# mbrzus/Cross-Modality-Minipig-Gan

Hardware: AMD Instinct MI355X
Metric: T1->T2 256x256 slices/sec (G+D step) (higher is better)
Workload: dtype f32

## Files before the change

cross-modality-minipig-gan_amd/csrc/conv_igemm.hip:

```cpp
#include "mpgan_common.h"
#include "conv_geom.h"
#include "lds_dma.h"
#include "conv_pipe.h"
#include <stdlib.h>
#include <algorithm>
#include <type_traits>

namespace mpgan {


struct KCursor {
  int ci, jz, jy, jx;
  int delta;
  int dz, dy, dx;
  int woff;
  bool valid;
};

template <int BN, int TM, int TN, int WN, bool SCALAR>
__global__ __launch_bounds__(256) void gather_conv_kernel(const GatherConv p) {
  extern __shared__ __attribute__((aligned(16))) float lds[];
  constexpr int STAGE = (BM + BN) * PITCH;
  constexpr int BROWS = BN / 32;

// ... 657 lines not shown
  const int T = p.Kz * p.Ky * p.Kx;
  for (int i = threadIdx.x; i < T * p.Cin; i += 256) wl[i] = p.wp[i];
  __syncthreads();
  const unsigned Mtot = (unsigned)p.N * ph.Mz * ph.My * ph.Mx;
  const unsigned gi = blockIdx.x * 256u + threadIdx.x;
  const unsigned m = gi / LANES;
  const int l = (int)(gi % LANES);
  const bool live = m < Mtot;
  PixDecode d = decode_pixel(p, ph, live ? m : 0u);
  float acc = 0.f;
  if (live && d.opix >= 0) {
    for (int jz = 0; jz < ph.nz; ++jz) {
      const int iz = d.bz + ph.dz0 + p.dstep[0] * jz, kz = ph.kz0 + p.kstep[0] * jz;
      if ((unsigned)iz >= (unsigned)p.Di) continue;
      for (int jy = 0; jy < ph.ny; ++jy) {
        const int iy = d.by + ph.dy0 + p.dstep[1] * jy, ky = ph.ky0 + p.kstep[1] * jy;
        if ((unsigned)iy >= (unsigned)p.Hi) continue;
        const long rowbase = (((long)d.n * p.Di + iz) * p.Hi + iy) * p.Wi;
        for (int jx = 0; jx < ph.nx; ++jx) {
          const int ix = d.bx + ph.dx0 + p.dstep[2] * jx, kx = ph.kx0 + p.kstep[2] * jx;
          if ((unsigned)ix >= (unsigned)p.Wi) continue;
          float4 v;
          if constexpr (IN_BF16) {
            typedef __bf16 bf16x4 __attribute__((ext_vector_type(4)));
            const bf16x4 t = *reinterpret_cast<const bf16x4*>(reinterpret_cast<const __bf16*>(p.in) + (rowbase + ix) * p.ldi + 4 * l);
            v = make_float4((float)t[0], (float)t[1], (float)t[2], (float)t[3]);
          } else {
            v = *reinterpret_cast<const float4*>(p.in + (rowbase + ix) * p.ldi + 4 * l);
          }
          const float4 w = *reinterpret_cast<const float4*>(wl + ((kz * p.Ky + ky) * p.Kx + kx) * p.Cin + 4 * l);
          acc = fmaf(v.x, w.x, acc);
          acc = fmaf(v.y, w.y, acc);
          acc = fmaf(v.z, w.z, acc);
          acc = fmaf(v.w, w.w, acc);
        }
      }
    }
  }
#pragma unroll
  for (int off = LANES / 2; off > 0; off >>= 1) acc += __shfl_xor(acc, off, 64);
  if (live && d.opix >= 0 && l == 0) {
    float v = acc + (p.bias ? p.bias[0] : 0.f);
    if (p.epi.scale) v = epi_act1(v, p.epi.scale[0], p.epi.shift[0], p.epi.slope[0]);
    if (p.resid) v += p.resid[(long)d.opix * p.ldr];
    if (p.tanh_out) v = tanhf(v);
    p.out[(long)d.opix * p.ldo] = v;
  }
}

template <int LANES>
__global__ __launch_bounds__(256) void convt_quad_cout1_kernel(const GatherConv p) {
  extern __shared__ __attribute__((aligned(16))) float wl[];
  const int Cin = p.Cin;
  for (int i = threadIdx.x; i < 9 * Cin; i += 256) wl[i] = p.wp[i];
  __syncthreads();
  const Phase& ph = p.ph[0];
  const unsigned Mtot = (unsigned)p.N * p.Hi * p.Wi;
  const unsigned gi = blockIdx.x * 256u + threadIdx.x;
  const unsigned m = gi / LANES;
  const int l = (int)(gi % LANES);
  const bool live = m < Mtot;
  unsigned q, ux, uy;
  fdivmod(live ? m : 0u, ph.fMx, q, ux);
  fdivmod(q, ph.fMy, q, uy);
  const int n = (int)q, y = (int)uy, x = (int)ux;
  const float* base = p.in + ((long)(n * p.Hi + y) * p.Wi + x) * p.ldi + 4 * l;
  const bool y1 = y + 1 < p.Hi, x1 = x + 1 < p.Wi;
  const float4 z4 = make_float4(0.f, 0.f, 0.f, 0.f);
  const float4 v00 = live ? *reinterpret_cast<const float4*>(base) : z4;
  const float4 v01 = live && x1 ? *reinterpret_cast<const float4*>(base + p.ldi) : z4;
  const float4 v10 = live && y1 ? *reinterpret_cast<const float4*>(base + (long)p.Wi * p.ldi) : z4;
  const float4 v11 = live && y1 && x1 ? *reinterpret_cast<const float4*>(base + (long)(p.Wi + 1) * p.ldi) : z4;
  auto W = [&](int ky, int kx) { return *reinterpret_cast<const float4*>(wl + (ky * 3 + kx) * Cin + 4 * l); };
  auto dot = [](const float4& a, const float4& b, float acc) {
    acc = fmaf(a.x, b.x, acc); acc = fmaf(a.y, b.y, acc); acc = fmaf(a.z, b.z, acc); return fmaf(a.w, b.w, acc);
  };
  float o00 = dot(v00, W(1, 1), 0.f);
  float o01 = dot(v01, W(1, 0), dot(v00, W(1, 2), 0.f));
  float o10 = dot(v10, W(0, 1), dot(v00, W(2, 1), 0.f));
  float o11 = dot(v11, W(0, 0), dot(v10, W(0, 2), dot(v01, W(2, 0), dot(v00, W(2, 2), 0.f))));
  const bool b0 = l & 1, b1 = l & 2;
  const float r0 = (b0 ? o10 : o00) + __shfl_xor(b0 ? o00 : o10, 1, 64);
  const float r1 = (b0 ? o11 : o01) + __shfl_xor(b0 ? o01 : o11, 1, 64);
  float t = (b1 ? r1 : r0) + __shfl_xor(b1 ? r0 : r1, 2, 64);
#pragma unroll
  for (int off = 4; off < LANES; off <<= 1) t += __shfl_xor(t, off, 64);
  float sv = 0.f;
  if (live && l < 4) {
    const int oy = 2 * y + (l & 1), ox = 2 * x + (l >> 1);
    if (oy < p.Ho && ox < p.Wo) {
      const long pix = ((long)n * p.Ho + oy) * p.Wo + ox;
      float v = t + (p.bias ? p.bias[0] : 0.f);
      sv = v;
      if (p.epi.scale) v = epi_act1(v, p.epi.scale[0], p.epi.shift[0], p.epi.slope[0]);
      if (p.resid) v += p.resid[pix * p.ldr];
      if (p.tanh_out) v = tanhf(v);
      p.out[pix * p.ldo] = v;
    }
  }
  if (p.stats || p.stats_acc) {
    __shared__ float ws1[4], ws2[4];
    const float s1 = wave_sum(sv), s2 = wave_sum(sv * sv);
    if ((threadIdx.x & 63) == 0) { ws1[threadIdx.x >> 6] = s1; ws2[threadIdx.x >> 6] = s2; }
    __syncthreads();
    if (threadIdx.x == 0) {
      const float t1 = ws1[0] + ws1[1] + ws1[2] + ws1[3], t2 = ws2[0] + ws2[1] + ws2[2] + ws2[3];
      if (p.stats_acc) {
        long long* rep = p.stats_acc + (long)(blockIdx.x % (unsigned)p.acc_rep) * ACC_WORDS;
        acc_add(rep, 1, 0, 0, t1);
        acc_add(rep, 1, 2, 0, t2);
      } else {
        p.stats[2 * (long)blockIdx.x] = t1;
        p.stats[2 * (long)blockIdx.x + 1] = t2;
      }
    }
  }
}

static bool convt_quad_ok(const GatherConv& p) {
  const int lanes = p.Cin / 4;
  if (!(p.Cout == 1 && !p.pro.scale && p.Cin % 4 == 0 && p.ldi % 4 == 0 && (lanes == 4 || lanes == 8 || lanes == 16) &&
        ((reinterpret_cast<uintptr_t>(p.in) & 15) == 0)))
    return false;
  if (!(p.nphase == 4 && p.Di == 1 && p.Do == 1 && p.Kz == 1 && p.Ky == 3 && p.Kx == 3 && p.ostride[1] == 2 &&
        p.ostride[2] == 2 && p.istride[1] == 1 && p.istride[2] == 1 && p.dstep[1] == -1 && p.dstep[2] == -1))
// ... 169 lines not shown
  const long obase = (((long)n * p.Do + z) * p.Ho + y) * p.Wo + x0;
  if (x0 + 3 < Mx && (p.Wo & 3) == 0 && ((reinterpret_cast<uintptr_t>(p.out) | reinterpret_cast<uintptr_t>(p.resid)) & 15) == 0) {
    float4 v = make_float4(o[0], o[1], o[2], o[3]);
    if (p.resid) {
      const float4 rr = *reinterpret_cast<const float4*>(p.resid + obase);
      v.x += rr.x; v.y += rr.y; v.z += rr.z; v.w += rr.w;
    }
    if (p.tanh_out) { v.x = tanhf(v.x); v.y = tanhf(v.y); v.z = tanhf(v.z); v.w = tanhf(v.w); }
    *reinterpret_cast<float4*>(p.out + obase) = v;
    return;
  }
#pragma unroll
  for (int j = 0; j < 4; ++j) {
    if (x0 + j >= Mx) break;
    float v = o[j];
    if (p.resid) v += p.resid[obase + j];
    if (p.tanh_out) v = tanhf(v);
    p.out[obase + j] = v;
  }
}

static bool thin_c1c1_ok(const GatherConv& p) {
  static const bool off = dev_env("MPGAN_DBG_NO_THIN_ROWS") != nullptr;
  if (off || !(p.Cin == 1 && p.Cout == 1 && p.ldi == 1 && p.ldo == 1 && (!p.resid || p.ldr == 1) && p.nphase == 1 &&
               !p.pro.scale && !p.stats && !p.stats_acc && !p.in_bf16 && !p.out_bf16 && !p.epi.scale && p.Ky == 3 && p.Kx == 3 &&
               (p.Kz == 3 || p.Kz == 1)))
    return false;
  const Phase& ph = p.ph[0];
  if (!(ph.ny == 3 && ph.nx == 3 && ph.nz == p.Kz && ph.oz == 0 && ph.oy == 0 && ph.ox == 0 && p.Do == ph.Mz &&
        p.Ho == ph.My && p.Wo == ph.Mx && p.Wi == ph.Mx && p.Hi == ph.My && p.Di == ph.Mz))
    return false;
  for (int d = 0; d < 3; ++d) {
    if (p.istride[d] != 1 || p.ostride[d] != 1) return false;
    if (d == 0 && p.Kz == 1) continue;
    const int d0 = d == 0 ? ph.dz0 : (d == 1 ? ph.dy0 : ph.dx0);
    if (!((p.dstep[d] == 1 && d0 == -1) || (p.dstep[d] == -1 && d0 == 1))) return false;
  }
  return true;
}

static bool thin_cin1_ok(const GatherConv& p) {
  const int T = p.Kz * p.Ky * p.Kx;
  return p.Cin == 1 && !p.pro.scale && (long)T * ((p.Cout + 3) / 4 * 4) * 4 <= 48 * 1024;
}

static bool thin_cout1_ok(const GatherConv& p) {
  const int T = p.Kz * p.Ky * p.Kx;
  const int lanes = p.Cin / 4;
  return p.Cout == 1 && !p.pro.scale && p.Cin % 4 == 0 && p.ldi % 4 == 0 && lanes >= 1 && lanes <= 64 &&
         (lanes & (lanes - 1)) == 0 && ((reinterpret_cast<uintptr_t>(p.in) & 15) == 0) &&
         (long)T * p.Cin * 4 <= 48 * 1024;
}

template <int T, bool OUT_BF16>
__global__ __launch_bounds__(256) void thin_cin1_rows_kernel(const GatherConv p) {
  __shared__ float red[4][128];
  constexpr int KZ = T == 27 ? 3 : 1;
  const Phase& ph = p.ph[0];
  const int lane = threadIdx.x & 63;
  const int wave = __builtin_amdgcn_readfirstlane((int)threadIdx.x >> 6);
  const int rows = p.N * ph.Mz * ph.My, Mx = ph.Mx;
  const int nwaves = (int)gridDim.x * 4, ngroups = (Mx + 3) >> 2;
  float w[T];
#pragma unroll
  for (int t = 0; t < T; ++t) w[t] = p.wp[(long)lane * T + t];
  const float bv = p.bias ? p.bias[lane] : 0.f;
  const bool act = OUT_BF16 && p.epi.scale != nullptr;
  const float esc = act ? p.epi.scale[lane] : 1.f, esh = act ? p.epi.shift[lane] : 0.f, esl = act ? p.epi.slope[lane] : 1.f;
  float s1 = 0.f, s2 = 0.f;
  for (int r = (int)blockIdx.x * 4 + wave; r < rows; r += nwaves) {
    const int my = r % ph.My, q = r / ph.My;
    const int mz = q % ph.Mz, n = q / ph.Mz;
    const float* __restrict__ g0 = p.in + (((long)n * p.Di + mz) * p.Hi + my) * p.Wi;
    const long orow = (long)r * Mx;
    for (int gi = 0; gi < ngroups; ++gi) {
      const int x0 = gi + 1 < ngroups ? 4 * gi : Mx - 4;
      const int first = 4 * gi - x0;
      float o[4] = {bv, bv, bv, bv};
#pragma unroll
      for (int kz = 0; kz < KZ; ++kz)
#pragma unroll
        for (int ky = 0; ky < 3; ++ky) {
          const float* __restrict__ src = g0 + ((long)kz * p.Hi + ky) * p.Wi + x0;
          float win[6];
#pragma unroll
          for (int i = 0; i < 6; ++i) win[i] = src[i];
#pragma unroll
          for (int kx = 0; kx < 3; ++kx)
#pragma unroll
            for (int j = 0; j < 4; ++j) o[j] = fmaf(w[(kz * 3 + ky) * 3 + kx], win[j + kx], o[j]);
        }
#pragma unroll
      for (int j = 0; j < 4; ++j) {
        const long e = (orow + x0 + j) * p.ldo + lane;
        if constexpr (OUT_BF16) reinterpret_cast<__bf16*>(p.out)[e] = (__bf16)(act ? epi_act1(o[j], esc, esh, esl) : o[j]);
        else p.out[e] = o[j];
        const float v = j >= first ? o[j] : 0.f;
        s1 += v;
        s2 = fmaf(v, v, s2);
      }
    }
  }
  if (p.stats) {
    red[wave][lane] = s1;
    red[wave][64 + lane] = s2;
    __syncthreads();
    if (threadIdx.x < 128)
      p.stats[(long)blockIdx.x * 128 + threadIdx.x] =
          (red[0][threadIdx.x] + red[1][threadIdx.x]) + (red[2][threadIdx.x] + red[3][threadIdx.x]);
  }
}

static bool thin_cin1_rows_ok(const GatherConv& p) {
  static const bool off = dev_env("MPGAN_DBG_NO_THIN_ROWS") != nullptr;
  const int T = p.Kz * p.Ky * p.Kx;
  const Phase& ph = p.ph[0];
  return !off && p.Cin == 1 && p.Cout == 64 && p.ldi == 1 && p.nphase == 1 && !p.pro.scale && !p.resid && !p.tanh_out &&
         !p.stats_acc && !p.in_bf16 && !p.epi.scale && (T == 9 || T == 27) && p.Kx == 3 && p.Ky == 3 && p.Kz == (T == 27 ? 3 : 1) &&
         ph.nx == 3 && ph.ny == 3 && ph.nz == p.Kz && ph.dx0 == 0 && ph.dy0 == 0 && ph.dz0 == 0 && ph.kx0 == 0 &&
         ph.ky0 == 0 && ph.kz0 == 0 && p.dstep[0] == 1 && p.dstep[1] == 1 && p.dstep[2] == 1 && p.kstep[0] == 1 &&
         p.kstep[1] == 1 && p.kstep[2] == 1 && p.istride[0] == 1 && p.istride[1] == 1 && p.istride[2] == 1 &&
         p.ostride[0] == 1 && p.ostride[1] == 1 && p.ostride[2] == 1 && ph.oz == 0 && ph.oy == 0 && ph.ox == 0 &&
         ph.Mx >= 4 && p.Wi == ph.Mx + 2 && p.Hi == ph.My + 2 && p.Di == ph.Mz + (T == 27 ? 2 : 0) && p.Wo == ph.Mx &&
         p.Ho == ph.My && p.Do == ph.Mz;
}

constexpr int PT_H = 8, PT_W = 16;
__device__ float g_patch_zero_page[64];

struct PatchLaunch {
  int tiles_x, tiles_y;
  int patch_floats;
  FastDiv fCout;
  FastDiv fPW[8], fNx[8];
  int merged, ylo, yhi, xlo, xhi, stats_off;
  FastDiv fPWm, fKx;
  int w_floats;
  int pca, pcw;
  const void* zero_page;
  FastDiv fTx, fTy;
  int stagger;
  int tw_off;
  int dbg;
};
static_assert(sizeof(GatherConv) + sizeof(PatchLaunch) <= 4096, "gather_patch kernel arguments exceed 4 KiB");

enum class GForm {
  ThinBf16OutRows,
  ThinBf16OutFull,
  ThinBf16InMfma,
  ThinBf16In,
  C1C1Rows4,
  Cin1Rows,
  Cin1Full,
  Cin1,
  ConvtQuad,
  ConvtOct,
  Cout1,
  Patch3d,
  Patch,
  PatchPersist,
  Mm16,
  Pipe,
  Dma,
  Kstep,
};

struct GatherChoice {
  GForm form;
  int rc;
  const char* msg;
  int code;
  int rows;
  int arg;
  int bn, wraps, pro, ks;
  bool fast;
  PatchLaunch pl;
  int smem, ntiles, grid;
};

template <int CIN, int PRO, bool NARROW, bool MERGE>
__global__ __launch_bounds__(256) void gather_patch_kernel(const GatherConv p, const PatchLaunch pl) {
  extern __shared__ __attribute__((aligned(16))) float lds[];
  typedef float f32x4 __attribute__((ext_vector_type(4)));
  constexpr int PC = CIN + 4;
  constexpr int CQ = CIN / 4;
  constexpr int LU = CIN == 16 ? 3 : (CIN == 32 ? 6 : 12);
  constexpr int WU = CIN == 16 ? 3 : (CIN == 32 ? 9 : 8);
  const int tid = threadIdx.x;
  const int lane = tid & 63, wid = tid >> 6;
  const unsigned wblk = xcd_remap(blockIdx.x, gridDim.x);
  const int phase0 = MERGE ? 0 : (int)(wblk % (unsigned)p.nphase);
  const int nph = MERGE ? p.nphase : 1;
  unsigned q = MERGE ? wblk : wblk / (unsigned)p.nphase;
  const int tx = (int)(q % (unsigned)pl.tiles_x);
  q /= (unsigned)pl.tiles_x;
  const int ty = (int)(q % (unsigned)pl.tiles_y);
  const int n = (int)(q / (unsigned)pl.tiles_y);
  const int Cout = p.Cout;
  const int my0 = ty * PT_H, mx0 = tx * PT_W;
  if constexpr (!MERGE) {
    const Phase& ph = p.ph[phase0];
    const int My = ph.Mz > 0 ? ph.My : 0, Mx = ph.Mx;
    if (my0 >= My || mx0 >= Mx) {
      if (p.stats && tid < Cout) {
        float* row = p.stats + (long)wblk * 2 * Cout;
        row[tid] = 0.f;
        row[Cout + tid] = 0.f;
      }
      return;
    }
// ... 1328 lines not shown
    }                                     \
  } while (0)

static GatherChoice choose_thin(const GatherConv& p, long maxM, GatherChoice c) {
  const int T = p.Kz * p.Ky * p.Kx;
  const long block_rows = (maxM + 255) / 256 * p.nphase;
  if (p.out_bf16) {
    CHOICE_REFUSE(!(thin_cin1_ok(p) && (p.Cout == 16 || p.Cout == 32 || p.Cout == 64) && p.ldo % 4 == 0 &&
                    (reinterpret_cast<uintptr_t>(p.out) & 7) == 0 && !p.resid && !p.tanh_out && !p.in_bf16 &&
                    (!p.bias || (reinterpret_cast<uintptr_t>(p.bias) & 15) == 0)),
                  "thin conv (bf16 out): needs Cin == 1, Cout in {16, 32, 64}, no resid/tanh, aligned output");
    CHOICE_REFUSE(p.stats && p.Cout > 64, "thin conv (bf16 out): fused statistics up to 64 channels");
    CHOICE_REFUSE(p.epi.scale && (p.stats || p.stats_acc), "thin conv (bf16 out): the epilogue activation goes without fused statistics");
    c.rows = (int)block_rows;
    GatherConv plain = p;
    plain.epi.scale = nullptr;
    if (thin_cin1_rows_ok(plain)) { c.form = GForm::ThinBf16OutRows; c.arg = T; return c; }
    c.form = GForm::ThinBf16OutFull;
    c.arg = p.Cout / 4;
    return c;
  }
  if (p.in_bf16) {
    if (thin_cout1_mfma_bf16_ok(p)) { c.form = GForm::ThinBf16InMfma; return c; }
    const int lanes_b = p.Cin / 4;
    CHOICE_REFUSE(!(p.Cout == 1 && !p.pro.scale && p.Cin % 4 == 0 && p.ldi % 4 == 0 &&
                    (lanes_b == 4 || lanes_b == 8 || lanes_b == 16) && (reinterpret_cast<uintptr_t>(p.in) & 7) == 0 &&
                    (long)T * p.Cin * 4 <= 48 * 1024 && !p.stats),
                  "thin conv (bf16 in): needs Cout == 1 and 16, 32 or 64 gathered channels");
    c.form = GForm::ThinBf16In;
    c.arg = lanes_b;
    return c;
  }
  if (thin_c1c1_ok(p)) { c.form = GForm::C1C1Rows4; c.arg = p.dstep[2] < 0; return c; }
  if (thin_cin1_ok(p)) {
    const bool v4 = (p.Cout % 4 == 0) && (p.ldo % 4 == 0) && ((reinterpret_cast<uintptr_t>(p.out) & 15) == 0);
    const bool full = v4 && (p.Cout == 16 || p.Cout == 32 || p.Cout == 64) &&
                      (!p.bias || (reinterpret_cast<uintptr_t>(p.bias) & 15) == 0) &&
                      (!p.resid || ((p.ldr % 4 == 0) && (reinterpret_cast<uintptr_t>(p.resid) & 15) == 0));
    CHOICE_REFUSE((p.stats || p.stats_acc) && !(full && p.Cout <= 32),
                  "thin conv: fused statistics need the all-channel kernel (Cout 16 or 32, 16-byte aligned output/bias)");
    if (full) {
      c.rows = (int)block_rows;
      if (!p.stats && thin_cin1_rows_ok(p)) { c.form = GForm::Cin1Rows; c.arg = T; return c; }
      c.form = GForm::Cin1Full;
      c.arg = p.Cout / 4;
      return c;
    }
    c.form = GForm::Cin1;
    c.arg = v4 ? 4 : 1;
    return c;
  }
  CHOICE_REFUSE((p.stats || p.stats_acc) && !convt_quad_ok(p),
                "thin conv: fused statistics of a 1-channel output exist for ConvTranspose2d(C -> 1, k3 s2) only");
  c.arg = p.Cin / 4;
  if (convt_quad_ok(p)) {
    c.form = GForm::ConvtQuad;
    c.rows = (int)(((long)p.N * p.Hi * p.Wi * c.arg + 255) / 256);
  } else {
    c.form = convt_oct_ok(p) ? GForm::ConvtOct : GForm::Cout1;
  }
  return c;
}

static GatherChoice choose_gather(const GatherConv& p, long maxM) {
  GatherChoice c{};
  c.rc = MPGAN_OK;
  if (p.out_bf16 || p.in_bf16) return choose_thin(p, maxM, c);
  const int variant = select_variant(p, maxM, thin_cin1_ok(p), thin_cout1_ok(p));
  c.code = c.bn = variant;
  CHOICE_REFUSE(p.epi.scale && (p.stats || p.stats_acc || p.bwd.part || p.fold.acc || p.ksplit > 1 || p.in_bf16 || p.out_bf16),
                "gather_conv: the epilogue activation goes with a plain forward (no fused statistics, split-K or bf16 storage)");
  CHOICE_REFUSE(p.fold.acc && (p.pro.n_stride != 0 || p.fold.cstride < p.Cin),
                "gather_conv: fold-on-load is per channel (BatchNorm) over >= Cin accumulator columns");
  if (variant <= 2) {
    CHOICE_REFUSE(p.fold.acc != nullptr, "thin conv: no fold-on-load");
    CHOICE_REFUSE(p.bwd.part != nullptr, "thin conv: no fused norm-backward sums (mpgan_conv_bwd_stats_rows() == 0)");
    return choose_thin(p, maxM, c);
  }
  if (patch3d_geom_ok(p)) {
    if (patch3d_operands_ok(p)) {
      static const bool no_mm16 = dev_env("MPGAN_DBG_NO_MM16") != nullptr;
      const P3Grid tg = patch3d_grid(p);
      c.form = GForm::Patch3d;
      c.code = 18;
      c.rows = p.N * tg.tiles_z * tg.tiles_y * tg.tiles_x;
      c.pro = p.pro.scale != nullptr;
      c.arg = p.mm16 && !no_mm16;
      return c;
    }
    CHOICE_REFUSE(p.stats != nullptr, "gather_conv: fused statistics of a 3-D patch-kernel geometry need 16-byte "
                                      "aligned operands, a channel pitch % 4 == 0 and < 2^31 input elements");
  }
  if (patch_plan(p, &c.pl, &c.smem)) {
    CHOICE_REFUSE(p.bwd.part != nullptr, "patch kernel: no fused norm-backward sums (mpgan_conv_bwd_stats_rows() == 0)");
    const bool aligned = (p.ldi % 4 == 0) && ((reinterpret_cast<uintptr_t>(p.in) & 15) == 0) &&
                         ((reinterpret_cast<uintptr_t>(p.wp) & 15) == 0) &&
                         (!p.pro.scale || ((reinterpret_cast<uintptr_t>(p.pro.scale) |
                                            reinterpret_cast<uintptr_t>(p.pro.shift)) & 15) == 0);
    if (aligned) {
      PatchLaunch pp;
      int psmem = 0;
      const bool persist = patch_persist_plan(p, c.pl, &pp, &psmem, &c.ntiles, &c.grid);
      CHOICE_REFUSE(!persist && (p.fold.acc || p.stats_acc),
                    "gather_patch: accumulator statistics / fold-on-load need the persistent patch kernel "
                    "(mpgan_conv_acc_supported / mpgan_conv_fold_supported said otherwise?)");
      c.code = c.pl.merged ? 17 : 16;
// ... 98 lines not shown
    }
    case GForm::C1C1Rows4: {
      const Phase& ph0 = p.ph[0];
      const long threads4 = (long)p.N * ph0.Mz * ph0.My * ((ph0.Mx + 3) / 4);
      if (c.arg) hipLaunchKernelGGL(thin_c1c1_rows4_kernel<true>, dim3((unsigned)((threads4 + 255) / 256)), dim3(256), 0, st, p);
      else hipLaunchKernelGGL(thin_c1c1_rows4_kernel<false>, dim3((unsigned)((threads4 + 255) / 256)), dim3(256), 0, st, p);
      return check_launch("thin_c1c1_rows4");
    }
    case GForm::Cin1Full: {
      const size_t smem = ((size_t)((T * p.Cout + 3) & ~3) + ((p.stats || p.stats_acc) ? 256 * (size_t)(p.Cout + 1) : 0)) * sizeof(float);
      if (c.arg == 4) hipLaunchKernelGGL(thin_cin1_full_kernel<4>, block_grid, dim3(256), smem, st, p);
      else if (c.arg == 8) hipLaunchKernelGGL(thin_cin1_full_kernel<8>, block_grid, dim3(256), smem, st, p);
      else hipLaunchKernelGGL(thin_cin1_full_kernel<16>, block_grid, dim3(256), smem, st, p);
      return check_launch("thin_cin1_full");
    }
    case GForm::Cin1: {
      const int CQ = (p.Cout + c.arg - 1) / c.arg;
      dim3 grid((unsigned)((maxM * CQ + 255) / 256), 1, (unsigned)p.nphase);
      const size_t smem = (size_t)T * CQ * c.arg * sizeof(float);
      if (c.arg == 4) hipLaunchKernelGGL(thin_cin1_kernel<4>, grid, dim3(256), smem, st, p);
      else hipLaunchKernelGGL(thin_cin1_kernel<1>, grid, dim3(256), smem, st, p);
      return check_launch("thin_cin1");
    }
    case GForm::ConvtQuad: {
      dim3 qgrid((unsigned)(((long)p.N * p.Hi * p.Wi * c.arg + 255) / 256));
      const size_t qsmem = (size_t)9 * p.Cin * sizeof(float);
      if (c.arg == 4) hipLaunchKernelGGL(convt_quad_cout1_kernel<4>, qgrid, dim3(256), qsmem, st, p);
      else if (c.arg == 8) hipLaunchKernelGGL(convt_quad_cout1_kernel<8>, qgrid, dim3(256), qsmem, st, p);
      else hipLaunchKernelGGL(convt_quad_cout1_kernel<16>, qgrid, dim3(256), qsmem, st, p);
      return check_launch("convt_quad_cout1");
    }
    case GForm::ConvtOct: {
      dim3 ogrid((unsigned)(((long)p.N * p.Di * p.Hi * p.Wi * c.arg + 255) / 256));
      const size_t osmem = (size_t)27 * p.Cin * sizeof(float);
      if (c.arg == 4) hipLaunchKernelGGL(convt_oct_cout1_kernel<4>, ogrid, dim3(256), osmem, st, p);
      else if (c.arg == 8) hipLaunchKernelGGL(convt_oct_cout1_kernel<8>, ogrid, dim3(256), osmem, st, p);
      else hipLaunchKernelGGL(convt_oct_cout1_kernel<16>, ogrid, dim3(256), osmem, st, p);
      return check_launch("convt_oct_cout1");
    }
    case GForm::Cout1: {
      dim3 grid((unsigned)((maxM * c.arg + 255) / 256), 1, (unsigned)p.nphase);
      const size_t smem = (size_t)T * p.Cin * sizeof(float);
      switch (c.arg) {
        case 1: hipLaunchKernelGGL(thin_cout1_kernel<1>, grid, dim3(256), smem, st, p); break;
        case 2: hipLaunchKernelGGL(thin_cout1_kernel<2>, grid, dim3(256), smem, st, p); break;
        case 4: hipLaunchKernelGGL(thin_cout1_kernel<4>, grid, dim3(256), smem, st, p); break;
        case 8: hipLaunchKernelGGL(thin_cout1_kernel<8>, grid, dim3(256), smem, st, p); break;
        case 16: hipLaunchKernelGGL(thin_cout1_kernel<16>, grid, dim3(256), smem, st, p); break;
        case 32: hipLaunchKernelGGL(thin_cout1_kernel<32>, grid, dim3(256), smem, st, p); break;
        default: hipLaunchKernelGGL(thin_cout1_kernel<64>, grid, dim3(256), smem, st, p); break;
      }
      return check_launch("thin_cout1");
    }
    case GForm::Patch3d: return launch_patch3d(p, c, st);
    case GForm::Patch:
      switch (p.Cin) {
        case 16: return launch_patch_cin<16>(p, c.pl, c.smem, st);
        case 32: return launch_patch_cin<32>(p, c.pl, c.smem, st);
        default: return launch_patch_cin<64>(p, c.pl, c.smem, st);
      }
    case GForm::PatchPersist: {
      static void* zp = nullptr;
      if (!zp && hipGetSymbolAddress(&zp, HIP_SYMBOL(g_patch_zero_page)) != hipSuccess) {
        zp = nullptr;
        set_error("gather_patch_persist: no address for the zero page");
        return MPGAN_ERR_HIP;
      }
      PatchLaunch pl = c.pl;
      pl.zero_page = zp;
      switch (p.Cin) {
        case 16: return launch_patch_persist_cin<16>(p, pl, c.smem, c.ntiles, c.grid, st);
        case 32: return launch_patch_persist_cin<32>(p, pl, c.smem, c.ntiles, c.grid, st);
        default: return launch_patch_persist_cin<64>(p, pl, c.smem, c.ntiles, c.grid, st);
      }
    }
    case GForm::Mm16: return launch_gather_mm16(p, c.bn, c.wraps, c.pro, c.ks, maxM, st);
    case GForm::Pipe: return c.wraps == 1 ? launch_pipe_pro<1>(p, c, maxM, st) : launch_pipe_pro<2>(p, c, maxM, st);
    case GForm::Dma:
      if (c.bn == 128) return launch_dma_variant<128, 2, 2, 2>(p, maxM, st);
      if (c.bn == 64) return launch_dma_variant<64, 1, 2, 1>(p, maxM, st);
      return launch_dma_variant<32, 1, 1, 1, 2>(p, maxM, st);
    case GForm::Kstep:
      if (c.arg) {
        if (c.bn == 128) return launch_variant<128, 2, 2, 2, true>(p, maxM, st);
        if (c.bn == 64) return launch_variant<64, 1, 2, 1, true>(p, maxM, st);
        return launch_variant<32, 1, 1, 1, true>(p, maxM, st);
      }
      if (c.bn == 128) return launch_variant<128, 2, 2, 2, false>(p, maxM, st);
      if (c.bn == 64) return launch_variant<64, 1, 2, 1, false>(p, maxM, st);
      return launch_variant<32, 1, 1, 1, false>(p, maxM, st);
  }
  return MPGAN_ERR_UNSUPPORTED;
}

static int gather_kernel_name(const GatherConv& p, const GatherChoice& c, char* buf, int len) {
  const char* b[2] = {"false", "true"};
  const int a = c.arg, lanes16 = a == 4 || a == 8 ? a : 16;
  const int T = p.Kz * p.Ky * p.Kx == 9 ? 9 : 27;
  const int tm = c.bn == 128 ? 2 : 1, tn = c.bn == 32 ? 1 : 2, wn = c.bn == 128 ? 2 : 1;
  const int cin = p.Cin == 16 || p.Cin == 32 ? p.Cin : 64;
  const int ppro = c.pl.merged ? 0 : c.pro;
  switch (c.form) {
    case GForm::ThinBf16OutRows: return snprintf(buf, len, "thin_cin1_rows_kernel<%d, true>", T);
    case GForm::Cin1Rows: return snprintf(buf, len, "thin_cin1_rows_kernel<%d, false>", T);
    case GForm::ThinBf16OutFull: return snprintf(buf, len, "thin_cin1_full_kernel<%d, true>", lanes16);
    case GForm::Cin1Full: return snprintf(buf, len, "thin_cin1_full_kernel<%d, false>", lanes16);
    case GForm::ThinBf16InMfma: return snprintf(buf, len, "thin_cout1_mfma_bf16_kernel");
    case GForm::ThinBf16In: return snprintf(buf, len, "thin_cout1_kernel<%d, true>", lanes16);
    case GForm::C1C1Rows4: return snprintf(buf, len, "thin_c1c1_rows4_kernel<%s>", b[a != 0]);
    case GForm::Cin1: return snprintf(buf, len, "thin_cin1_kernel<%d>", a == 4 ? 4 : 1);
    case GForm::ConvtQuad: return snprintf(buf, len, "convt_quad_cout1_kernel<%d>", lanes16);
    case GForm::ConvtOct: return snprintf(buf, len, "convt_oct_cout1_kernel<%d>", lanes16);
    case GForm::Cout1:
      return snprintf(buf, len, "thin_cout1_kernel<%d, false>", a > 0 && a <= 32 && (a & (a - 1)) == 0 ? a : 64);
    case GForm::Patch3d: return snprintf(buf, len, "gather_patch3d_c16_kernel<%s, %s>", b[c.pro != 0], b[a != 0]);
    case GForm::Patch:
    case GForm::PatchPersist:
      return snprintf(buf, len, "%s<%d, %d, %s, %s>",
                      c.form == GForm::Patch ? "gather_patch_kernel" : "gather_patch_persist_kernel", cin, ppro,
                      b[p.Cout <= 16], b[c.pl.merged != 0]);
    case GForm::Mm16: {
      const int ks = c.wraps == 1 && c.ks == 2 && c.bn != 128 ? 2 : 1;
      return snprintf(buf, len, "gather_conv_pipe_kernel<%d, %d, %d, %d, %d, %d, false, %d, true>", c.bn, tm, tn, wn,
                      c.wraps, c.pro, ks);
    }
    case GForm::Pipe: {
      const bool fast = c.wraps == 1 && c.pro == 3 && c.fast;
      const int ks = !fast && c.wraps == 1 && c.pro != 3 && c.ks == 2 ? 2 : 1;
      const int bn = fast ? 128 : (ks == 2 && c.bn != 64 ? 32 : c.bn);
      return snprintf(buf, len, "gather_conv_pipe_kernel<%d, %d, %d, %d, %d, %d, %s, %d, false>", bn,
                      bn == 128 ? 2 : 1, bn == 32 ? 1 : 2, bn == 128 ? 2 : 1, c.wraps, c.pro, b[fast], ks);
    }
    case GForm::Dma: return snprintf(buf, len, "gather_conv_dma_kernel<%d, %d, %d, %d, 2>", c.bn, tm, tn, wn);
    case GForm::Kstep: return snprintf(buf, len, "gather_conv_kernel<%d, %d, %d, %d, %s>", c.bn, tm, tn, wn, b[a != 0]);
  }
  return snprintf(buf, len, "?");
}

#ifdef MPGAN_STAMPS
static int launch_gather_impl(const GatherConv& p, hipStream_t st);
static int launch_gather(const GatherConv& p0, hipStream_t st) {
  GatherConv p = p0;
  StampCtx& c = stamp_ctx();
  p.stamps = nullptr;
  p.stamp_blocks = 0;
  if (c.base && c.next < c.launches) {
    p.stamps = c.base + c.next * c.blocks * MPGAN_STAMP_SLOTS;
    p.stamp_blocks = (int)c.blocks;
    c.next += 1;
  }
  return launch_gather_impl(p, st);
}
static int launch_gather_impl(const GatherConv& p, hipStream_t st) {
#else
static int launch_gather(const GatherConv& p, hipStream_t st) {
#endif
  const long maxM = max_phase_pixels(p);
  if (maxM == 0) return MPGAN_OK;
  MPGAN_CHECK_ARG((long)p.N * p.Do * p.Ho * p.Wo < (1L << 31) && (long)p.N * p.Di * p.Hi * p.Wi < (1L << 31) &&
                      maxM < (1L << 31) - 256,
                  "gather_conv: more than 2^31 pixels");
  MPGAN_CHECK_ARG((long)p.Cout * p.Cin * p.Kz * p.Ky * p.Kx < (1L << 31), "gather_conv: weight larger than 2^31");
  return launch_chosen(p, choose_gather(p, maxM), maxM, st);
}

}

// ... 322 lines not shown
```

cross-modality-minipig-gan_amd/csrc/conv_wgrad.hip:

```cpp
#include "mpgan_common.h"
#include <stdlib.h>
#include <type_traits>

#include "wgrad_pipe.h"

namespace mpgan {

template <int BD, int BG, int TM, int TN, int WN, int KW, bool SCALAR_D, bool SCALAR_G>
__global__ __launch_bounds__(256) void wgrad_kernel(const WgradParams p) {
  extern __shared__ __attribute__((aligned(16))) float lds[];
  constexpr int STAGE = WBK * (BD + BG);
  constexpr int DCH = BD / 4, GCH = BG / 4;
  constexpr int DLOADS = (WBK * DCH) / 256;
  constexpr int GLOADS = (WBK * GCH) / 256 > 0 ? (WBK * GCH) / 256 : 1;
  constexpr int GTHREADS = WBK * GCH;

  const int tid = threadIdx.x;
  const int lane = tid & 63, wid = tid >> 6;
  const int li = lane & 31, lh = lane >> 5;
  const int wm = KW == 1 ? wid / WN : 0, wn = KW == 1 ? wid % WN : 0;
  const int T = p.Kz * p.Ky * p.Kx;
  const int NC = T * p.Cg;
  const WBlockId bid = wgrad_block_id(p);
  const int c0 = bid.tc * BG;
// ... 300 lines not shown
    const int tt = (int)(rem / Cg);
    const int cg = (int)(rem - (long)tt * Cg);
    const long o = (cd * Cg + cg) * T + tt;
    dw[o] = beta != 0.f ? beta * dw[o] + t : t;
  }
}

static inline void launch_wgrad_reduce(hipStream_t st, const float* partial, float* dw, int nsplit, int Cd, int Cg, int T,
                                       float beta, const float* bp, int bsplit, float* db) {
  const long total = (long)Cd * Cg * T;
  if (total <= 32L * 512 && nsplit >= 64) {
    const int blocks = (int)((total + 7) / 8), bb = db ? (Cd + 7) / 8 : 0;
    hipLaunchKernelGGL(wgrad_reduce_narrow_kernel, dim3(blocks + bb), dim3(256), 0, st, partial, dw, nsplit, Cd, Cg, T, beta,
                       bp, bsplit, db, bb);
    return;
  }
  int blocks = (int)((total + 31) / 32);
  if (blocks > 8192) blocks = 8192;
  const int bb = db ? (Cd + 31) / 32 : 0;
  hipLaunchKernelGGL(wgrad_reduce_kernel, dim3(blocks + bb), dim3(256), 0, st, partial, dw, nsplit, Cd, Cg, T, beta, bp,
                     bsplit, db, bb);
}

__global__ __launch_bounds__(256) void wgrad_bias_reduce_kernel(const float* __restrict__ bp, int nsplit, int Cd,
                                                                float* __restrict__ db, float beta) {
  const int gt = blockIdx.x * blockDim.x + threadIdx.x;
  const int c = gt >> 6, lane = threadIdx.x & 63;
  if (c >= Cd) return;
  double s = 0.0;
  for (int k = lane; k < nsplit; k += 64) s += (double)bp[(long)k * Cd + c];
#pragma unroll
  for (int off = 32; off > 0; off >>= 1) s += __shfl_xor(s, off, 64);
  if (lane == 0) db[c] = beta != 0.f ? beta * db[c] + (float)s : (float)s;
}

template <int V, int T, bool DENSE_BF16 = false>
__global__ __launch_bounds__(256) void wgrad_thin_kernel(const WgradParams p) {
  extern __shared__ float red[];
  const int CQ = (p.Cd + V - 1) / V;
  const int PL = 256 / CQ;
  const int q = threadIdx.x % CQ, pl = threadIdx.x / CQ;
  const int c = q * V;
  const long M = (long)p.N * p.Mz * p.My * p.Mx;
  const long mbeg = (long)blockIdx.x * p.chunk;
  const long mend = mbeg + p.chunk < M ? mbeg + p.chunk : M;
  float acc[T][V], bsum[V];
#pragma unroll
  for (int t = 0; t < T; ++t)
#pragma unroll
    for (int e = 0; e < V; ++e) acc[t][e] = 0.f;
#pragma unroll
  for (int e = 0; e < V; ++e) bsum[e] = 0.f;
  if (pl < PL) {
    for (long m = mbeg + pl; m < mend; m += PL) {
      unsigned r, umx, umy, umz;
      fdivmod((unsigned)m, p.fMx, r, umx);
      fdivmod(r, p.fMy, r, umy);
      fdivmod(r, p.fMz, r, umz);
      const int mx = (int)umx, my = (int)umy, mz = (int)umz, n = (int)r;
      float d[V];
      if constexpr (DENSE_BF16) {
        typedef __bf16 bf16x4 __attribute__((ext_vector_type(4)));
        const bf16x4 t4 = *reinterpret_cast<const bf16x4*>(reinterpret_cast<const __bf16*>(p.dense) + m * p.ldd + c);
#pragma unroll
        for (int e = 0; e < V; ++e) d[e] = (float)t4[e < 4 ? e : 0];
      } else if (V == 4 && c + 3 < p.Cd) {
        const float4 t4 = *reinterpret_cast<const float4*>(p.dense + m * p.ldd + c);
        d[0] = t4.x; d[V > 1 ? 1 : 0] = t4.y; d[V > 2 ? 2 : 0] = t4.z; d[V > 3 ? 3 : 0] = t4.w;
      } else {
#pragma unroll
        for (int e = 0; e < V; ++e) d[e] = c + e < p.Cd ? p.dense[m * p.ldd + c + e] : 0.f;
      }
#pragma unroll
      for (int e = 0; e < V; ++e) bsum[e] += d[e];
      const int bz = mz * p.sz - p.pz, by = my * p.sy - p.py, bx = mx * p.sx - p.px;
      const float* __restrict__ g0 = p.gath + ((((long)n * p.Gz + bz) * p.Gy + by) * p.Gx + bx) * p.ldg;
      constexpr int KX = T == 1 ? 1 : 3, KY = KX, KZ = T / (KX * KY);
#pragma unroll
      for (int kz = 0; kz < KZ; ++kz) {
        const bool okz = (unsigned)(bz + kz) < (unsigned)p.Gz;
#pragma unroll
        for (int ky = 0; ky < KY; ++ky) {
          const bool oky = okz && (unsigned)(by + ky) < (unsigned)p.Gy;
          const int ro = (kz * p.Gy + ky) * p.Gx * p.ldg;
#pragma unroll
          for (int kx = 0; kx < KX; ++kx) {
            const int t = (kz * KY + ky) * KX + kx;
            const bool ok = oky && (unsigned)(bx + kx) < (unsigned)p.Gx;
            const float g = ok ? g0[ro + kx * p.ldg] : 0.f;
#pragma unroll
            for (int e = 0; e < V; ++e) acc[t][e] = fmaf(d[e], g, acc[t][e]);
          }
        }
      }
    }
  }
  const int W = p.Cd * T + p.Cd;
  const int NR = p.fold_rounds > 1 ? p.fold_rounds : 1;
  const int PLr = PL / NR;
  for (int r = 0; r < NR; ++r) {
    if (pl < PLr * NR && pl / PLr == r) {
      const int row = pl - r * PLr;
#pragma unroll
      for (int e = 0; e < V; ++e) {
        if (c + e >= p.Cd) break;
#pragma unroll
        for (int t = 0; t < T; ++t) {
          float* dst = red + row * W + (c + e) * T + t;
          *dst = r == 0 ? acc[t][e] : *dst + acc[t][e];
        }
        float* db = red + row * W + p.Cd * T + c + e;
        *db = r == 0 ? bsum[e] : *db + bsum[e];
      }
    }
    __syncthreads();
  }
  const int PLf = PLr;
  float* out = p.partial + (long)blockIdx.x * p.Cd * T;
  const int G = W < 128 ? 256 / W : 1;
  if (G > 1) {
    const int i = threadIdx.x % W, g = threadIdx.x / W;
    const int GR = G < PLf ? G : PLf;
    float s1 = 0.f;
    if (g < GR)
      for (int r = g; r < PLf; r += GR) s1 += red[r * W + i];
    __syncthreads();
    if (g < GR) red[g * W + i] = s1;
    __syncthreads();
  }
  const int rows = G > 1 ? (G < PLf ? G : PLf) : PLf;
  for (int i = threadIdx.x; i < W; i += 256) {
    float s2 = 0.f;
    for (int r = 0; r < rows; ++r) s2 += red[r * W + i];
    if (i < p.Cd * T) out[i] = s2;
    else if (p.bias_partial) p.bias_partial[(long)blockIdx.x * p.Cd + (i - p.Cd * T)] = s2;
  }
}

template <int T, bool DENSE_BF16>
__global__ __launch_bounds__(256) void wgrad_thin_rows_kernel(const WgradParams p) {
  __shared__ float red[4][64 * T + 64];
  constexpr int KZ = T == 27 ? 3 : 1;
  const int lane = threadIdx.x & 63;
  const int wave = __builtin_amdgcn_readfirstlane((int)threadIdx.x >> 6);
  const int rows = p.N * p.Mz * p.My;
  const int nwaves = (int)gridDim.x * 4;
// ... 940 lines not shown
```

Measured before the change: 295.0.

## Add MFMA kernel for Cin64-to-Cout1 conv, batch wgrad loads, hoist convt loads

Adds an MFMA-based kernel for 64-to-1 channel convolutions. It computes per-tap partial products for an input tile with 16x16x4 f32 MFMAs into LDS, then sums the shifted taps per output pixel. The thin weight-gradient kernel now issues loads for four positions before accumulating, to raise memory-level parallelism. The ConvTranspose quad kernel issues its global input loads before the weight staging barrier so their latency overlaps it. The costs are more LDS, more registers, and more unconditional loads, which rely on clamped in-bounds addresses.

```diff
diff --git a/cross-modality-minipig-gan_amd/csrc/conv_igemm.hip b/cross-modality-minipig-gan_amd/csrc/conv_igemm.hip
--- a/cross-modality-minipig-gan_amd/csrc/conv_igemm.hip
+++ b/cross-modality-minipig-gan_amd/csrc/conv_igemm.hip
@@ -733,8 +733,6 @@
 __global__ __launch_bounds__(256) void convt_quad_cout1_kernel(const GatherConv p) {
   extern __shared__ __attribute__((aligned(16))) float wl[];
   const int Cin = p.Cin;
-  for (int i = threadIdx.x; i < 9 * Cin; i += 256) wl[i] = p.wp[i];
-  __syncthreads();
   const Phase& ph = p.ph[0];
   const unsigned Mtot = (unsigned)p.N * p.Hi * p.Wi;
   const unsigned gi = blockIdx.x * 256u + threadIdx.x;
@@ -748,10 +746,17 @@
   const float* base = p.in + ((long)(n * p.Hi + y) * p.Wi + x) * p.ldi + 4 * l;
   const bool y1 = y + 1 < p.Hi, x1 = x + 1 < p.Wi;
   const float4 z4 = make_float4(0.f, 0.f, 0.f, 0.f);
-  const float4 v00 = live ? *reinterpret_cast<const float4*>(base) : z4;
-  const float4 v01 = live && x1 ? *reinterpret_cast<const float4*>(base + p.ldi) : z4;
-  const float4 v10 = live && y1 ? *reinterpret_cast<const float4*>(base + (long)p.Wi * p.ldi) : z4;
-  const float4 v11 = live && y1 && x1 ? *reinterpret_cast<const float4*>(base + (long)(p.Wi + 1) * p.ldi) : z4;
+  const long ox1 = x1 ? p.ldi : 0, oy1 = y1 ? (long)p.Wi * p.ldi : 0;
+  float4 v00 = *reinterpret_cast<const float4*>(base);
+  float4 v01 = *reinterpret_cast<const float4*>(base + ox1);
+  float4 v10 = *reinterpret_cast<const float4*>(base + oy1);
+  float4 v11 = *reinterpret_cast<const float4*>(base + oy1 + ox1);
+  for (int i = threadIdx.x; i < 9 * Cin; i += 256) wl[i] = p.wp[i];
+  __syncthreads();
+  if (!live) v00 = z4;
+  if (!(live && x1)) v01 = z4;
+  if (!(live && y1)) v10 = z4;
+  if (!(live && y1 && x1)) v11 = z4;
   auto W = [&](int ky, int kx) { return *reinterpret_cast<const float4*>(wl + (ky * 3 + kx) * Cin + 4 * l); };
   auto dot = [](const float4& a, const float4& b, float acc) {
     acc = fmaf(a.x, b.x, acc); acc = fmaf(a.y, b.y, acc); acc = fmaf(a.z, b.z, acc); return fmaf(a.w, b.w, acc);
@@ -1027,6 +1032,146 @@
          (long)T * p.Cin * 4 <= 48 * 1024;
 }
 
+struct TcfGrid { int tz, ty, tx, tiles_z, tiles_y, tiles_x, pitch; };
+static_assert(sizeof(GatherConv) + sizeof(TcfGrid) <= 4096, "thin_cout1_mfma kernel arguments exceed 4 KiB");
+
+template <int NB>
+__global__ __launch_bounds__(256) void thin_cout1_mfma_kernel(const GatherConv p, const TcfGrid tg) {
+  extern __shared__ __attribute__((aligned(16))) float Pl[];
+  typedef float f32x4 __attribute__((ext_vector_type(4)));
+  const Phase& ph = p.ph[0];
+  const int tid = threadIdx.x, lane = tid & 63, wid = tid >> 6;
+  const int l16 = lane & 15, kq = lane >> 4;
+  const int T = ph.nz * ph.ny * ph.nx;
+  int t = blockIdx.x;
+  const int bx = t % tg.tiles_x; t /= tg.tiles_x;
+  const int by = t % tg.tiles_y; t /= tg.tiles_y;
+  const int bz = t % tg.tiles_z;
+  const int n = t / tg.tiles_z;
+  const int oz0 = bz * tg.tz, oy0 = by * tg.ty, ox0 = bx * tg.tx;
+  const int mnz = ph.dz0 + (p.dstep[0] < 0 ? (ph.nz - 1) * p.dstep[0] : 0), mny = ph.dy0 + (p.dstep[1] < 0 ? (ph.ny - 1) * p.dstep[1] : 0),
+            mnx = ph.dx0 + (p.dstep[2] < 0 ? (ph.nx - 1) * p.dstep[2] : 0);
+  const int PZ = tg.tz + ph.nz - 1, PY = tg.ty + ph.ny - 1, PX = tg.tx + ph.nx - 1;
+  const int NQ = PZ * PY * PX;
+
+  float w[NB][16];
+#pragma unroll
+  for (int b = 0; b < NB; ++b) {
+    const int tap = 16 * b + l16;
+    const bool tv = tap < T;
+    const int jx = tv ? tap % ph.nx : 0, tq = tv ? tap / ph.nx : 0, jy = tq % ph.ny, jz = tq / ph.ny;
+    const int kz = ph.kz0 + p.kstep[0] * jz, ky = ph.ky0 + p.kstep[1] * jy, kx = ph.kx0 + p.kstep[2] * jx;
+    const float* wrow = p.wp + (long)((kz * p.Ky + ky) * p.Kx + kx) * 64 + 4 * kq;
+#pragma unroll
+    for (int s = 0; s < 4; ++s) {
+      const float4 v = tv ? *reinterpret_cast<const float4*>(wrow + 16 * s) : make_float4(0.f, 0.f, 0.f, 0.f);
+      w[b][4 * s] = v.x; w[b][4 * s + 1] = v.y; w[b][4 * s + 2] = v.z; w[b][4 * s + 3] = v.w;
+    }
+  }
+  const float* __restrict__ gin = p.in;
+  auto load_group = [&](int rb, float4 (&a)[4]) {
+    const int q = rb * 16 + l16;
+    const int pz = q / (PY * PX), rem = q - pz * (PY * PX), py = rem / PX, px = rem - py * PX;
+    const int iz = oz0 + mnz + pz, iy = oy0 + mny + py, ix = ox0 + mnx + px;
+    const bool ok = q < NQ && (unsigned)iz < (unsigned)p.Di && (unsigned)iy < (unsigned)p.Hi && (unsigned)ix < (unsigned)p.Wi;
+    const float* src = gin + ((((long)n * p.Di + iz) * p.Hi + iy) * p.Wi + ix) * p.ldi + 4 * kq;
+#pragma unroll
+    for (int s = 0; s < 4; ++s) a[s] = ok ? *reinterpret_cast<const float4*>(src + 16 * s) : make_float4(0.f, 0.f, 0.f, 0.f);
+  };
+  float4 a[4], an[4] = {};
+  if (wid * 16 < NQ) load_group(wid, a);
+  for (int rb = wid; rb * 16 < NQ; rb += 4) {
+    if ((rb + 4) * 16 < NQ) load_group(rb + 4, an);
+    f32x4 acc[NB];
+#pragma unroll
+    for (int b = 0; b < NB; ++b) acc[b] = f32x4{0.f, 0.f, 0.f, 0.f};
+#pragma unroll
+    for (int s = 0; s < 4; ++s)
+#pragma unroll
+      for (int b = 0; b < NB; ++b) {
+        acc[b] = __builtin_amdgcn_mfma_f32_16x16x4f32(a[s].x, w[b][4 * s], acc[b], 0, 0, 0);
+        acc[b] = __builtin_amdgcn_mfma_f32_16x16x4f32(a[s].y, w[b][4 * s + 1], acc[b], 0, 0, 0);
+        acc[b] = __builtin_amdgcn_mfma_f32_16x16x4f32(a[s].z, w[b][4 * s + 2], acc[b], 0, 0, 0);
+        acc[b] = __builtin_amdgcn_mfma_f32_16x16x4f32(a[s].w, w[b][4 * s + 3], acc[b], 0, 0, 0);
+      }
+#pragma unroll
+    for (int b = 0; b < NB; ++b)
+      if (16 * b + l16 < T)
+        *reinterpret_cast<float4*>(Pl + (16 * b + l16) * tg.pitch + rb * 16 + 4 * kq) =
+            make_float4(acc[b][0], acc[b][1], acc[b][2], acc[b][3]);
+#pragma unroll
+    for (int s = 0; s < 4; ++s) a[s] = an[s];
+  }
+  __syncthreads();
+  const int lx = tid % tg.tx, lq = tid / tg.tx, ly = lq % tg.ty, lz = lq / tg.ty;
+  const int oz = oz0 + lz, oy = oy0 + ly, ox = ox0 + lx;
+  if (lz < tg.tz && oz < ph.Mz && oy < ph.My && ox < ph.Mx) {
+    float sum = 0.f;
+    int j = 0;
+    for (int jz = 0; jz < ph.nz; ++jz) {
+      const int qz = lz + ph.dz0 + p.dstep[0] * jz - mnz;
+      for (int jy = 0; jy < ph.ny; ++jy) {
+        const int qy = ly + ph.dy0 + p.dstep[1] * jy - mny;
+        for (int jx = 0; jx < ph.nx; ++jx, ++j) {
+          const int qx = lx + ph.dx0 + p.dstep[2] * jx - mnx;
+          sum += Pl[j * tg.pitch + (qz * PY + qy) * PX + qx];
+        }
+      }
+    }
+    p.out[(long)(((n * p.Do + oz) * p.Ho + oy) * p.Wo + ox) * p.ldo] = sum;
+  }
+}
+
+static bool thin_cout1_mfma_ok(const GatherConv& p) {
+  static const bool off = dev_env("MPGAN_DBG_NO_TC_MFMA") != nullptr;
+  if (off || p.in_bf16 || p.out_bf16 || p.Cout != 1 || p.Cin != 64 || p.nphase != 1 || p.bias || p.resid || p.tanh_out ||
+      p.stats || p.stats_acc || p.pro.scale || p.epi.scale || p.ldi % 4 != 0 ||
+      ((reinterpret_cast<uintptr_t>(p.in) | reinterpret_cast<uintptr_t>(p.wp)) & 15))
+    return false;
+  const Phase& ph = p.ph[0];
+  if (ph.nz < 1 || ph.ny < 1 || ph.nx < 1 || ph.nz > 3 || ph.ny > 3 || ph.nx > 3) return false;
+  for (int d = 0; d < 3; ++d)
+    if (p.istride[d] != 1 || p.ostride[d] != 1 || (p.dstep[d] != 1 && p.dstep[d] != -1)) return false;
+  if (ph.oz || ph.oy || ph.ox || ph.Mz != p.Do || ph.My != p.Ho || ph.Mx != p.Wo) return false;
+  return (long)p.N * p.Do * p.Ho * p.Wo * p.ldo < (1L << 31);
+}
+
+static TcfGrid thin_cout1_mfma_grid(const GatherConv& p) {
+  const Phase& ph = p.ph[0];
+  TcfGrid tg;
+  if (ph.nz == 1) { tg.tz = 1; tg.ty = 16; tg.tx = 16; }
+  else { tg.tz = 4; tg.ty = 8; tg.tx = 8; }
+  tg.tiles_z = (ph.Mz + tg.tz - 1) / tg.tz;
+  tg.tiles_y = (ph.My + tg.ty - 1) / tg.ty;
+  tg.tiles_x = (ph.Mx + tg.tx - 1) / tg.tx;
+  const int nq = (tg.tz + ph.nz - 1) * (tg.ty + ph.ny - 1) * (tg.tx + ph.nx - 1);
+  tg.pitch = (nq + 15) / 16 * 16;
+  while (tg.pitch % 64 != 16) tg.pitch += 16;
+  return tg;
+}
+
+static int launch_thin_cout1_mfma(const GatherConv& p, hipStream_t st) {
+  const Phase& ph = p.ph[0];
+  const TcfGrid tg = thin_cout1_mfma_grid(p);
+  const int T = ph.nz * ph.ny * ph.nx;
+  const int smem = T * tg.pitch * (int)sizeof(float);
+  static bool attr_set = false;
+  if (!attr_set) {
+    hipError_t e = hipFuncSetAttribute(reinterpret_cast<const void*>(thin_cout1_mfma_kernel<2>),
+                                       hipFuncAttributeMaxDynamicSharedMemorySize, 27 * 656 * (int)sizeof(float));
+    if (e != hipSuccess) {
+      set_error("thin_cout1_mfma: hipFuncSetAttribute: %s", hipGetErrorString(e));
+      return MPGAN_ERR_HIP;
+    }
+    attr_set = true;
+  }
+  const long blocks = (long)p.N * tg.tiles_z * tg.tiles_y * tg.tiles_x;
+  MPGAN_CHECK_ARG(blocks < (1L << 31), "thin_cout1_mfma: too many tiles");
+  if (T <= 16) hipLaunchKernelGGL(thin_cout1_mfma_kernel<1>, dim3((unsigned)blocks), dim3(256), smem, st, p, tg);
+  else hipLaunchKernelGGL(thin_cout1_mfma_kernel<2>, dim3((unsigned)blocks), dim3(256), smem, st, p, tg);
+  return check_launch("thin_cout1_mfma");
+}
+
 template <int T, bool OUT_BF16>
 __global__ __launch_bounds__(256) void thin_cin1_rows_kernel(const GatherConv p) {
   __shared__ float red[4][128];
@@ -1132,6 +1277,7 @@
   ConvtQuad,
   ConvtOct,
   Cout1,
+  Cout1Mfma,
   Patch3d,
   Patch,
   PatchPersist,
@@ -2566,6 +2712,7 @@
   }
   CHOICE_REFUSE((p.stats || p.stats_acc) && !convt_quad_ok(p),
                 "thin conv: fused statistics of a 1-channel output exist for ConvTranspose2d(C -> 1, k3 s2) only");
+  if (thin_cout1_mfma_ok(p)) { c.form = GForm::Cout1Mfma; c.arg = p.ph[0].nz * p.ph[0].ny * p.ph[0].nx <= 16 ? 1 : 2; return c; }
   c.arg = p.Cin / 4;
   if (convt_quad_ok(p)) {
     c.form = GForm::ConvtQuad;
@@ -2770,6 +2917,7 @@
       }
       return check_launch("thin_cout1");
     }
+    case GForm::Cout1Mfma: return launch_thin_cout1_mfma(p, st);
     case GForm::Patch3d: return launch_patch3d(p, c, st);
     case GForm::Patch:
       switch (p.Cin) {
@@ -2831,6 +2979,7 @@
     case GForm::ConvtOct: return snprintf(buf, len, "convt_oct_cout1_kernel<%d>", lanes16);
     case GForm::Cout1:
       return snprintf(buf, len, "thin_cout1_kernel<%d, false>", a > 0 && a <= 32 && (a & (a - 1)) == 0 ? a : 64);
+    case GForm::Cout1Mfma: return snprintf(buf, len, "thin_cout1_mfma_kernel<%d>", a);
     case GForm::Patch3d: return snprintf(buf, len, "gather_patch3d_c16_kernel<%s, %s>", b[c.pro != 0], b[a != 0]);
     case GForm::Patch:
     case GForm::PatchPersist:
diff --git a/cross-modality-minipig-gan_amd/csrc/conv_wgrad.hip b/cross-modality-minipig-gan_amd/csrc/conv_wgrad.hip
--- a/cross-modality-minipig-gan_amd/csrc/conv_wgrad.hip
+++ b/cross-modality-minipig-gan_amd/csrc/conv_wgrad.hip
@@ -376,46 +376,64 @@
 #pragma unroll
   for (int e = 0; e < V; ++e) bsum[e] = 0.f;
   if (pl < PL) {
-    for (long m = mbeg + pl; m < mend; m += PL) {
-      unsigned r, umx, umy, umz;
-      fdivmod((unsigned)m, p.fMx, r, umx);
-      fdivmod(r, p.fMy, r, umy);
-      fdivmod(r, p.fMz, r, umz);
-      const int mx = (int)umx, my = (int)umy, mz = (int)umz, n = (int)r;
-      float d[V];
-      if constexpr (DENSE_BF16) {
-        typedef __bf16 bf16x4 __attribute__((ext_vector_type(4)));
-        const bf16x4 t4 = *reinterpret_cast<const bf16x4*>(reinterpret_cast<const __bf16*>(p.dense) + m * p.ldd + c);
-#pragma unroll
-        for (int e = 0; e < V; ++e) d[e] = (float)t4[e < 4 ? e : 0];
-      } else if (V == 4 && c + 3 < p.Cd) {
-        const float4 t4 = *reinterpret_cast<const float4*>(p.dense + m * p.ldd + c);
-        d[0] = t4.x; d[V > 1 ? 1 : 0] = t4.y; d[V > 2 ? 2 : 0] = t4.z; d[V > 3 ? 3 : 0] = t4.w;
-      } else {
-#pragma unroll
-        for (int e = 0; e < V; ++e) d[e] = c + e < p.Cd ? p.dense[m * p.ldd + c + e] : 0.f;
-      }
-#pragma unroll
-      for (int e = 0; e < V; ++e) bsum[e] += d[e];
-      const int bz = mz * p.sz - p.pz, by = my * p.sy - p.py, bx = mx * p.sx - p.px;
-      const float* __restrict__ g0 = p.gath + ((((long)n * p.Gz + bz) * p.Gy + by) * p.Gx + bx) * p.ldg;
-      constexpr int KX = T == 1 ? 1 : 3, KY = KX, KZ = T / (KX * KY);
-#pragma unroll
-      for (int kz = 0; kz < KZ; ++kz) {
-        const bool okz = (unsigned)(bz + kz) < (unsigned)p.Gz;
-#pragma unroll
-        for (int ky = 0; ky < KY; ++ky) {
-          const bool oky = okz && (unsigned)(by + ky) < (unsigned)p.Gy;
-          const int ro = (kz * p.Gy + ky) * p.Gx * p.ldg;
-#pragma unroll
-          for (int kx = 0; kx < KX; ++kx) {
-            const int t = (kz * KY + ky) * KX + kx;
-            const bool ok = oky && (unsigned)(bx + kx) < (unsigned)p.Gx;
-            const float g = ok ? g0[ro + kx * p.ldg] : 0.f;
-#pragma unroll
-            for (int e = 0; e < V; ++e) acc[t][e] = fmaf(d[e], g, acc[t][e]);
+    constexpr int U = T == 27 ? 1 : 4;
+    constexpr int KX = T == 1 ? 1 : 3, KY = KX, KZ = T / (KX * KY);
+    for (long m0 = mbeg + pl; m0 < mend; m0 += (long)U * PL) {
+      float d[U][V], g[U][T];
+#pragma unroll
+      for (int u = 0; u < U; ++u) {
+        const long mu = m0 + (long)u * PL;
+        const bool live = mu < mend;
+        const long m = live ? mu : m0;
+        unsigned r, umx, umy, umz;
+        fdivmod((unsigned)m, p.fMx, r, umx);
+        fdivmod(r, p.fMy, r, umy);
+        fdivmod(r, p.fMz, r, umz);
+        const int mx = (int)umx, my = (int)umy, mz = (int)umz, n = (int)r;
+        if constexpr (DENSE_BF16) {
+          typedef __bf16 bf16x4 __attribute__((ext_vector_type(4)));
+          const bf16x4 t4 = *reinterpret_cast<const bf16x4*>(reinterpret_cast<const __bf16*>(p.dense) + m * p.ldd + c);
+#pragma unroll
+          for (int e = 0; e < V; ++e) d[u][e] = live ? (float)t4[e < 4 ? e : 0] : 0.f;
+        } else if constexpr (V == 4) {
+          float4 t4 = *reinterpret_cast<const float4*>(p.dense + m * p.ldd + c);
+          if (!live) t4 = make_float4(0.f, 0.f, 0.f, 0.f);
+          d[u][0] = t4.x; d[u][V > 1 ? 1 : 0] = t4.y; d[u][V > 2 ? 2 : 0] = t4.z; d[u][V > 3 ? 3 : 0] = t4.w;
+        } else {
+          static_assert(V == 1 || V == 4, "wgrad_thin_kernel: one channel or four per thread");
+          const float dv = p.dense[m * p.ldd + c];
+          d[u][0] = live ? dv : 0.f;
+        }
+        const int bz = mz * p.sz - p.pz, by = my * p.sy - p.py, bx = mx * p.sx - p.px;
+        const float* __restrict__ g0 = p.gath + ((((long)n * p.Gz + bz) * p.Gy + by) * p.Gx + bx) * p.ldg;
+#pragma unroll
+        for (int kz = 0; kz < KZ; ++kz) {
+          const bool okz = live && (unsigned)(bz + kz) < (unsigned)p.Gz;
+#pragma unroll
+          for (int ky = 0; ky < KY; ++ky) {
+            const bool oky = okz && (unsigned)(by + ky) < (unsigned)p.Gy;
+            const int ro = (kz * p.Gy + ky) * p.Gx * p.ldg;
+#pragma unroll
+            for (int kx = 0; kx < KX; ++kx) {
+              const bool ok = oky && (unsigned)(bx + kx) < (unsigned)p.Gx;
+              if constexpr (U > 1) {
+                const float gv = *(ok ? g0 + (ro + kx * p.ldg) : p.gath);
+                g[u][(kz * KY + ky) * KX + kx] = ok ? gv : 0.f;
+              } else {
+                g[u][(kz * KY + ky) * KX + kx] = ok ? g0[ro + kx * p.ldg] : 0.f;
+              }
+            }
           }
         }
+      }
+#pragma unroll
+      for (int u = 0; u < U; ++u) {
+#pragma unroll
+        for (int e = 0; e < V; ++e) bsum[e] += d[u][e];
+#pragma unroll
+        for (int t = 0; t < T; ++t)
+#pragma unroll
+          for (int e = 0; e < V; ++e) acc[t][e] = fmaf(d[u][e], g[u][t], acc[t][e]);
       }
     }
   }
```

After: 297.0 (median of 6 runs). No clear change (+0.7%).
